# wenhao728/VORTA

Measured on AMD Instinct MI355X. Metric: video_tokens_per_sec (routed-attention denoising step, HunyuanVideo 720p 129f), higher is better.
Workload: dtype fp16

## Files before the change

include/vorta_hip.h:

```cpp
#ifndef VORTA_HIP_H
#define VORTA_HIP_H

#include <stdint.h>

#ifdef __cplusplus
extern "C" {
#endif

#define VORTA_OK 0
#define VORTA_EINVAL (-1)
#define VORTA_EUNSUPPORTED (-2)
#define VORTA_ELAUNCH (-3)

#define VORTA_ABI_VERSION 9

typedef enum vorta_dtype {
  VORTA_BF16 = 0,
  VORTA_FP16 = 1,
  VORTA_FP32 = 2,
  VORTA_FP8E4M3 = 3,
  VORTA_INT8 = 4
} vorta_dtype;

typedef struct vorta_tensor {
// ... 16 lines not shown
  int32_t n_kv, kv_row_offset;
  const int32_t* kv_rows;
  int64_t kv_rows_stride_h, kv_rows_stride_g;
  const int32_t* dup_rows;
  int64_t dup_rows_stride_h;
  int32_t n_dup_pos, n_dup;
  float scale;
  int32_t block_rows;
  int32_t n_splits;
  float* ws_o;
  float* ws_ml;
  const int32_t* n_kv_dev;
  const int32_t* q_valid_dev;
  int32_t variant;
  int32_t reserved;
  const int32_t* q_block_table;
  int32_t n_q_blocks;
  int32_t reserved2;
} vorta_attn_args;

int vorta_attn_fwd(const vorta_attn_args* args, void* hip_stream);
#define VORTA_MAX_FUSED_LAUNCHES 6
int vorta_attn_fwd_batch(const vorta_attn_args* args, int32_t n, void* hip_stream);
int vorta_attn_plan(const vorta_attn_args* args, int32_t* block_rows, int64_t* n_workgroups, int32_t* kernel_id);
int vorta_attn_workspace_bytes(const vorta_attn_args* args, uint64_t* ws_o_bytes, uint64_t* ws_ml_bytes);

typedef struct vorta_attn_bwd_args {
  uint32_t struct_size;
  int32_t reserved;
  vorta_attn_args fwd;
  vorta_tensor d_o;
  const void* do_scale;
  int64_t do_scale_stride_h;
  vorta_tensor dq, dk, dv;
} vorta_attn_bwd_args;

int vorta_attn_bwd(const vorta_attn_bwd_args* args, void* hip_stream);

typedef struct vorta_attn_bwd_kmajor_args {
  uint32_t struct_size;
  int32_t n_key_lists;
  vorta_attn_bwd_args bwd;
  float* stats;
  int64_t stats_stride_h;
} vorta_attn_bwd_kmajor_args;

// ... 317 lines not shown
```

vorta_amd/_C.py:

```python
import ctypes as C
import os

_HERE = os.path.dirname(os.path.abspath(__file__))
LIB_PATH = os.environ.get("VORTA_HIP_LIB") or os.path.join(_HERE, "csrc", "libvorta_hip.so")

VORTA_OK, VORTA_EINVAL, VORTA_EUNSUPPORTED, VORTA_ELAUNCH = 0, -1, -2, -3
VORTA_BF16, VORTA_FP16, VORTA_FP32, VORTA_FP8E4M3, VORTA_INT8 = 0, 1, 2, 3, 4
ABI_VERSION = 9

_i32, _i64, _u32, _f32, _vp = C.c_int32, C.c_int64, C.c_uint32, C.c_float, C.c_void_p


class Tensor(C.Structure):
    _fields_ = [("ptr", _vp), ("stride_h", _i64), ("stride_s", _i64)]


class AttnArgs(C.Structure):
    _fields_ = [
        ("struct_size", _u32), ("dtype", _i32), ("head_dim", _i32), ("n_heads", _i32),
        ("q", Tensor), ("k", Tensor), ("v", Tensor), ("o", Tensor),
        ("head_list", _vp), ("n_heads_dev", _vp),
        ("n_q", _i32), ("q_group_len", _i32), ("q_row_offset", _i32), ("q_valid", _i32),
        ("q_rows", _vp), ("q_rows_stride_h", _i64),
        ("n_kv", _i32), ("kv_row_offset", _i32),
# ... 162 lines not shown
        ("rows", _vp), ("win", _vp), ("keep_rows", _vp), ("keep_rows_stride_h", _i64),
        ("drop_rows", _vp), ("drop_rows_stride_h", _i64), ("head_list", _vp), ("n_heads_dev", _vp),
    ]


MIX_BWD_PARTS = 64
NORM_ROPE_BWD_PARTS = 1024
FIDELITY_PARTS, FIDELITY_WS_FLOATS = 64, 12


def fidelity_chain(n_rows: int) -> int:
    return ((n_rows + FIDELITY_PARTS - 1) // FIDELITY_PARTS + 15) // 16 + 21

SAMPLED_FIDELITY_PARTS, SAMPLED_FIDELITY_WS_FLOATS, SAMPLED_FIDELITY_ROW_CHAIN = 16, 8, 11


def sampled_fidelity_chain(n_rows: int) -> int:
    return ((n_rows + SAMPLED_FIDELITY_PARTS - 1) // SAMPLED_FIDELITY_PARTS + 15) // 16 + 19


SYMBOLS = {
    "vorta_attn_fwd": (C.c_int, [C.POINTER(AttnArgs), _vp]),
    "vorta_attn_fwd_batch": (C.c_int, [C.POINTER(AttnArgs), _i32, _vp]),
    "vorta_attn_plan": (C.c_int, [C.POINTER(AttnArgs), C.POINTER(_i32), C.POINTER(_i64), C.POINTER(_i32)]),
    "vorta_attn_workspace_bytes": (C.c_int, [C.POINTER(AttnArgs), C.POINTER(C.c_uint64), C.POINTER(C.c_uint64)]),
    "vorta_fp8_quant_ws_floats": (C.c_int, [_i32, _i32]),
    "vorta_fp8_quant_ws_partials": (C.c_int, [_i32, _i32, C.POINTER(_i64), C.POINTER(_i64)]),
    "vorta_fp8_quantize_qkv": (C.c_int, [C.POINTER(Fp8QuantArgs), _vp]),
    "vorta_fp8_v_absmax": (C.c_int, [C.POINTER(Fp8VArgs), _vp]),
    "vorta_fp8_v_convert": (C.c_int, [C.POINTER(Fp8VArgs), _vp]),
    "vorta_attn_fwd_fp8": (C.c_int, [C.POINTER(AttnArgs), C.POINTER(AttnFp8Ext), _vp]),
    "vorta_attn_fwd_batch_fp8": (C.c_int, [C.POINTER(AttnArgs), C.POINTER(AttnFp8Ext), _i32, _vp]),
    "vorta_i8_quantize_k": (C.c_int, [C.POINTER(I8QuantArgs), _vp]),
    "vorta_i8_tail_flags": (C.c_int, [C.POINTER(Tensor), _i32, _i32, _vp, C.c_float, _vp, _vp]),
    "vorta_split_heads": (C.c_int, [_vp, _vp, _i32, _vp, _vp, _vp, _vp, _vp]),
    "vorta_attn_fwd_i8": (C.c_int, [C.POINTER(AttnArgs), C.POINTER(AttnI8Ext), _vp]),
    "vorta_attn_fwd_batch_i8": (C.c_int, [C.POINTER(AttnArgs), C.POINTER(AttnI8Ext), _i32, _vp]),
    "vorta_coreset_select": (C.c_int, [C.POINTER(CoresetArgs), _vp]),
    "vorta_sta_table_sizes": (C.c_int, [C.POINTER(StaArgs), C.POINTER(_i32), C.POINTER(_i32), C.POINTER(_i32)]),
    "vorta_sta_build_tables": (C.c_int, [C.POINTER(StaArgs), _vp]),
    "vorta_coreset_select_partial": (C.c_int, [C.POINTER(CoresetArgs), _vp]),
    "vorta_sta_partial_sizes": (C.c_int, [C.POINTER(StaArgs), C.POINTER(_i32), C.POINTER(_i32), C.POINTER(_i32),
                                          C.POINTER(_i32), _i32]),
    "vorta_sta_build_tables_partial": (C.c_int, [C.POINTER(StaArgs), _vp]),
    "vorta_router_route": (C.c_int, [C.POINTER(RouterArgs), _vp]),
    "vorta_route_scores": (C.c_int, [C.POINTER(RouterArgs), _vp]),
# ... 88 lines not shown
```

vorta_amd/_debug.py:

```python
import os

KEYS = ("coreset_kv_order", "fused_text_splits", "sta_merge", "fp8_center_k", "joint_projection", "attn_variant", "no_xcd_remap",
        "sp_staging", "sp_group_streams", "sp_v_wire", "sp_emulate_link_gbps")


def _parse(text: str) -> dict:
    out = {}
    for item in filter(None, (x.strip() for x in text.split(","))):
        key, _, value = item.partition("=")
        if key not in KEYS:
            raise ValueError(f"VORTA_DEBUG: unknown key {key!r} (one of {KEYS})")
        out[key] = value if value else "1"
    return out


FLAGS = _parse(os.environ.get("VORTA_DEBUG", ""))


def flag(key: str, default: str) -> str:
    if key not in KEYS:
        raise KeyError(key)
    return FLAGS.get(key, default)
```

vorta_amd/csrc/attn_common.h:

```cpp
#pragma once
#include <hip/hip_runtime.h>
#include <stdint.h>

#include "vorta_hip.h"
#include "common.h"

namespace vorta_attn {


constexpr int KVB = 64;
constexpr int D = 128;
constexpr int ROWB = D * 2;
constexpr int TILE_BYTES = KVB * ROWB;
constexpr int BUF_BYTES = 2 * TILE_BYTES;

struct Params {
  const char* q; const char* k; const char* v; char* o;
  int64_t q_sh, k_sh, v_sh, o_sh;
  int64_t q_ss, k_ss, v_ss, o_ss;
  const int32_t* head_list; const int32_t* n_heads_dev;
  int n_heads;
  int n_q, q_group_len, q_row_offset, q_valid;
  int n_groups, blocks_per_group;
  const int32_t* q_rows; int64_t q_rows_sh;
// ... 24 lines not shown
__device__ __forceinline__ int live_order(const Params& p, int b, int n, bool remap) {
  if (p.n_heads_dev) n = min(n, max(*p.n_heads_dev, 0) * p.wg_per_slot);
  if (!remap || b >= n) return b;
  const int xcd = b & 7, qd = n >> 3, r = n & 7;
  return (xcd < r ? xcd * (qd + 1) : r * (qd + 1) + (xcd - r) * qd) + (b >> 3);
}

#ifndef VORTA_MAX_SEGMENTS
#define VORTA_MAX_SEGMENTS VORTA_MAX_FUSED_LAUNCHES
#endif
constexpr int MAX_SEGMENTS = VORTA_MAX_SEGMENTS;
template <class PP> __host__ __device__ __forceinline__ Params& base_of(PP& pp) { return pp.p; }
template <class PP> __host__ __device__ __forceinline__ const Params& base_of(const PP& pp) { return pp.p; }
__host__ __device__ __forceinline__ Params& base_of(Params& p) { return p; }
__host__ __device__ __forceinline__ const Params& base_of(const Params& p) { return p; }

template <class PP> struct MultiOf {
  PP seg[MAX_SEGMENTS];
  int start[MAX_SEGMENTS + 1];
  int n;
};

template <class PP>
__device__ __forceinline__ const PP& segment_of(const MultiOf<PP>& mp, int b, int& wg) {
  int s = 0;
#pragma unroll
  for (int i = 1; i < MAX_SEGMENTS; ++i) s += (i < mp.n && b >= mp.start[i]) ? 1 : 0;
  wg = live_order(base_of(mp.seg[s]), b - mp.start[s], mp.start[s + 1] - mp.start[s], true);
  return mp.seg[s];
}

__device__ __forceinline__ float2 out_descale(const Params&, int, int) { return make_float2(1.f, 1.f); }
template <class PP> __device__ __forceinline__ float2 out_descale(const PP& pp, int head, int lane) {
  return *(const float2*)(pp.v_descale + (int64_t)head * pp.v_descale_sh + lane * 2);
}

template <typename T, class PP>
__global__ __launch_bounds__(256) void attn_combine_kernel(const PP pp) {
  const Params& p = base_of(pp);
  const int lane = threadIdx.x & 63;
  const int64_t item = (int64_t)blockIdx.x * 4 + (threadIdx.x >> 6);
  if (item >= (int64_t)p.n_heads * p.n_q) return;
  const int y = (int)(item / p.n_q);
  const int pos = (int)(item - (int64_t)y * p.n_q);
  if (p.n_heads_dev && y >= *p.n_heads_dev) return;
  const int head = p.head_list ? p.head_list[y] : y;
  float m = -1e30f;
  for (int s = 0; s < p.n_splits; ++s) m = fmaxf(m, p.ws_ml[(((int64_t)y * p.n_splits + s) * p.n_q + pos) * 2]);
  float acc0 = 0.f, acc1 = 0.f, l = 0.f;
  for (int s = 0; s < p.n_splits; ++s) {
    const int64_t slot = ((int64_t)y * p.n_splits + s) * p.n_q + pos;
    const float w = __builtin_amdgcn_exp2f(p.ws_ml[slot * 2] - m);
// ... 36 lines not shown
int launch_single(void (*kernel)(PP), int block_rows, const PP& pp, hipStream_t st) {
  const Params& p = base_of(pp);
  const int64_t total = (int64_t)p.n_groups * p.blocks_per_group * p.n_heads * p.n_splits;
  if (total <= 0) return VORTA_OK;
  if (total > 0x7fffffff) return VORTA_EINVAL;
  hipLaunchKernelGGL(kernel, dim3((unsigned)total), dim3(block_rows * 2), 0, st, pp);
  const hipError_t e = hipGetLastError();
  if (e != hipSuccess) return vorta_set_hip_error(e);
  return launch_combine<T>(pp, st);
}

template <class F>
int fwd_single(const F& f, const vorta_attn_args* a, void* hip_stream) {
  typename F::PP pp{};
  int block_rows = 0;
  const int rc = f.fill(a, pp, block_rows);
  if (rc != VORTA_OK) return rc;
  if (base_of(pp).n_heads == 0 || base_of(pp).n_groups == 0) return VORTA_OK;
  hipStream_t st = (hipStream_t)hip_stream;
  if (f.out_dtype(*a) == VORTA_BF16) return launch_single<__bf16>(F::template kernel<__bf16>(*a, pp, block_rows), block_rows, pp, st);
  return launch_single<_Float16>(F::template kernel<_Float16>(*a, pp, block_rows), block_rows, pp, st);
}

template <typename T, class PP>
int launch_fused(void (*kernel)(MultiOf<PP>), const MultiOf<PP>& mp, int total, hipStream_t st) {
  hipLaunchKernelGGL(kernel, dim3((unsigned)total), dim3(512), 0, st, mp);
  const hipError_t e = hipGetLastError();
  if (e != hipSuccess) return vorta_set_hip_error(e);
  for (int i = 0; i < mp.n; ++i) {
    const int rc = launch_combine<T>(mp.seg[i], st);
    if (rc != VORTA_OK) return rc;
  }
  return VORTA_OK;
}

template <class F>
int fwd_batch(const F& f, const vorta_attn_args* args, int32_t n, void* hip_stream) {
  if (!args || n < 0 || n > MAX_SEGMENTS) return VORTA_EINVAL;
  MultiOf<typename F::PP> mp{};
  int64_t total = 0;
  int dtype = -1, m = 0;
  for (int i = 0; i < n; ++i) {
    typename F::PP pp{};
    int block_rows = 0;
    const int rc = f.fill(&args[i], pp, block_rows);
    if (rc != VORTA_OK) return rc;
    Params& p = base_of(pp);
    if (p.n_heads == 0 || p.n_groups == 0) continue;
    if (block_rows != 256 || !f.fusable(args[i], pp)) return VORTA_EUNSUPPORTED;
    if (dtype >= 0 && dtype != f.out_dtype(args[i])) return VORTA_EINVAL;
    dtype = f.out_dtype(args[i]);
    p.xcd_remap = 0;
    mp.seg[m] = pp;
    mp.start[m] = (int)total;
    total += (int64_t)p.n_groups * p.blocks_per_group * p.n_heads * p.n_splits;
    if (total > 0x7fffffff) return VORTA_EINVAL;
    ++m;
  }
  if (m == 0) return VORTA_OK;
  for (int i = m; i <= MAX_SEGMENTS; ++i) mp.start[i] = (int)total;
  mp.n = m;
  hipStream_t st = (hipStream_t)hip_stream;
  if (dtype == VORTA_BF16) return launch_fused<__bf16>(F::template multi<__bf16>, mp, (int)total, st);
  return launch_fused<_Float16>(F::template multi<_Float16>, mp, (int)total, st);
}

int fill_params(const vorta_attn_args* a, Params& p, int& block_rows, int in_esize, int v_esize = 0, int k_esize = 0);
int mx_fwd(const vorta_attn_args* a, const vorta_attn_fp8_ext* ext, void* hip_stream);
int mx_fwd_batch(const vorta_attn_args* args, const vorta_attn_fp8_ext* ext, int32_t n, void* hip_stream);

template <typename T> struct MF;
template <> struct MF<__bf16> {
  using v8 = bf16x8; using v4 = bf16x4;
  static __device__ __forceinline__ f32x16 mfma(v8 a, v8 b, f32x16 c) {
    return __builtin_amdgcn_mfma_f32_32x32x16_bf16(a, b, c, 0, 0, 0);
  }
  static __device__ __forceinline__ v4 tr(const char* p) {
    return __builtin_amdgcn_ds_read_tr16_b64_v4bf16((LDS_AS v4*)p);
  }
};
template <> struct MF<_Float16> {
  using v8 = f16x8; using v4 = f16x4;
  static __device__ __forceinline__ f32x16 mfma(v8 a, v8 b, f32x16 c) {
    return __builtin_amdgcn_mfma_f32_32x32x16_f16(a, b, c, 0, 0, 0);
  }
  static __device__ __forceinline__ v4 tr(const char* p) {
    typedef __attribute__((ext_vector_type(4))) __fp16 h4;
// ... 17 lines not shown
```

vorta_amd/csrc/attn_fwd.hip:

```cpp
#include <hip/hip_runtime.h>
#include <stdint.h>

#include "vorta_hip.h"
#include "common.h"

#include "attn_common.h"
#include "attn_fwd_diag.inc"

namespace {
using namespace vorta_attn;

template <typename T, int NW>
__global__ __launch_bounds__(NW * 64, 2) void attn_fwd_kernel(const Params p) {
  using V8 = typename MF<T>::v8;
  using V4 = typename MF<T>::v4;
  constexpr int NT = NW * 64;
  constexpr int QB = NW * 32;
  constexpr int CH = (KVB * 16) / NT;
  constexpr int ROWSTEP = NT / 16;

  __shared__ __attribute__((aligned(16))) char smem[2 * BUF_BYTES];

  const int wg = live_order(p, blockIdx.x, gridDim.x, p.xcd_remap);
  const int sp = wg % p.n_splits;
  const int rest = wg / p.n_splits;
  const int n_qb = p.n_groups * p.blocks_per_group;
  const int qb = rest % n_qb;
  const int y = rest / n_qb;
  if (p.n_heads_dev && y >= *p.n_heads_dev) return;
  const int head = p.head_list ? p.head_list[y] : y;
  int grp, p0, pend;
  q_block_of(p, qb, QB, grp, p0, pend);

  const int tid = threadIdx.x;
  const int lane = tid & 63;
  const int wave = __builtin_amdgcn_readfirstlane(tid >> 6);
  const int r32 = lane & 31;
  const int hh = lane >> 5;

  const int n_kv = p.n_kv_dev ? max(1, min(*p.n_kv_dev, p.n_kv)) : p.n_kv;
  const int q_valid = p.q_valid_dev ? min(*p.q_valid_dev, p.q_valid) : p.q_valid;
  const int nblk_total = (n_kv + KVB - 1) / KVB;
  const int blk0 = sp * p.blocks_per_split;
  const int blk1 = min(blk0 + p.blocks_per_split, nblk_total);

  const int wrow0 = p0 + wave * 32;
  const bool wave_active = wrow0 < pend;
  const int my_p = wrow0 + r32;
  const bool row_ok = my_p < pend;
  const int ld_p = min(my_p, pend - 1);
  const int32_t* q_rows = p.q_rows ? p.q_rows + (int64_t)y * p.q_rows_sh : nullptr;
  const int64_t my_row = q_rows ? (int64_t)q_rows[ld_p] : (int64_t)(p.q_row_offset + ld_p);

  V8 qf[8];
  {
    const char* qp = p.q + (int64_t)head * p.q_sh + my_row * p.q_ss + hh * 16;
#pragma unroll
    for (int ks = 0; ks < 8; ++ks) qf[ks] = *(const V8*)(qp + ks * 32);
  }

  const int32_t* kv_rows =
      p.kv_rows ? p.kv_rows + (int64_t)y * p.kv_rows_sh + (int64_t)grp * p.kv_rows_sg : nullptr;
  const char* kbase = p.k + (int64_t)head * p.k_sh + (tid & 15) * 16;
  const char* vbase = p.v + (int64_t)head * p.v_sh + (tid & 15) * 16;
  const int lrow0 = tid >> 4;
  const int lcc = tid & 15;
  int k_wr[CH], v_wr[CH];
#pragma unroll
  for (int i = 0; i < CH; ++i) {
    const int row = lrow0 + i * ROWSTEP;
// ... 31 lines not shown

  f32x16 o[4];
#pragma unroll
  for (int dt = 0; dt < 4; ++dt)
#pragma unroll
    for (int i = 0; i < 16; ++i) o[dt][i] = 0.f;
  float m_run = -1e30f, l_run = 0.f;
  const float c = p.scale_log2;

  if (blk0 < blk1) {
    FETCH_ROWS(blk0);
    ISSUE_LOADS();
    if (blk0 + 1 < blk1) { FETCH_ROWS(blk0 + 1); }
    WRITE_LDS(0);
    if (blk0 + 1 < blk1) { ISSUE_LOADS(); }
    if (blk0 + 2 < blk1) { FETCH_ROWS(blk0 + 2); }
    __syncthreads();
  }

  for (int blk = blk0; blk < blk1; ++blk) {
    const int buf = (blk - blk0) & 1;
    const char* sb = smem + buf * BUF_BYTES;
    V8 pb[4];
    if (wave_active) {
      f32x16 s0, s1;
#pragma unroll
      for (int i = 0; i < 16; ++i) { s0[i] = 0.f; s1[i] = 0.f; }
#pragma unroll
      for (int ks = 0; ks < 8; ++ks) {
        const V8 k0 = *(const V8*)(sb + k_rd[ks]);
        const V8 k1 = *(const V8*)(sb + k_rd[ks] + 32 * ROWB);
        s0 = MF<T>::mfma(k0, qf[ks], s0);
        s1 = MF<T>::mfma(k1, qf[ks], s1);
      }
      const int kv0 = blk * KVB;
      if (kv0 + KVB > n_kv) {
#pragma unroll
        for (int i = 0; i < 16; ++i) {
          const int row = (i & 3) + 8 * (i >> 2) + 4 * hh;
          if (kv0 + row >= n_kv) s0[i] = -INFINITY;
          if (kv0 + 32 + row >= n_kv) s1[i] = -INFINITY;
        }
      }
      float mx = s0[0];
#pragma unroll
      for (int i = 1; i < 16; ++i) mx = fmaxf(mx, s0[i]);
#pragma unroll
// ... 11 lines not shown
      }
      const float mc = m_run * c;
      float lsum = 0.f;
#pragma unroll
      for (int i = 0; i < 16; ++i) {
        s0[i] = __builtin_amdgcn_exp2f(fmaf(s0[i], c, -mc));
        s1[i] = __builtin_amdgcn_exp2f(fmaf(s1[i], c, -mc));
        lsum += s0[i] + s1[i];
      }
      l_run += lsum;
#pragma unroll
      for (int j = 0; j < 8; ++j) {
        pb[0][j] = (T)s0[j];
        pb[1][j] = (T)s0[8 + j];
        pb[2][j] = (T)s1[j];
        pb[3][j] = (T)s1[8 + j];
      }
    }
    if (blk + 1 < blk1) {
      WRITE_LDS(buf ^ 1);
      if (blk + 2 < blk1) { ISSUE_LOADS(); }
      if (blk + 3 < blk1) { FETCH_ROWS(blk + 3); }
    }
    if (wave_active) {
#pragma unroll
      for (int dt = 0; dt < 4; ++dt) {
#pragma unroll
        for (int kg = 0; kg < 4; ++kg) {
          const V4 lo = MF<T>::tr(sb + v_rd[dt] + (16 * kg) * ROWB);
          const V4 hi = MF<T>::tr(sb + v_rd[dt] + (16 * kg + 8) * ROWB);
          V8 vf;
#pragma unroll
          for (int j = 0; j < 4; ++j) { vf[j] = lo[j]; vf[4 + j] = hi[j]; }
          o[dt] = MF<T>::mfma(vf, pb[kg], o[dt]);
        }
      }
    }
    __syncthreads();
  }

  if (!wave_active) return;
  const float l_tot = half_sum(l_run);
  if (p.n_splits > 1) {
    if (row_ok) {
      const int64_t slot = ((int64_t)y * p.n_splits + sp) * p.n_q + my_p;
      float* wo = p.ws_o + slot * D;
#pragma unroll
// ... 40 lines not shown

constexpr int RING = 2;

template <typename T, int NW, bool KVTAB, int NS>
__device__ __forceinline__ void attn_pipe_dma_body(const Params& p, char* __restrict__ smem, const int wg) {
  static_assert(NS == 2, "ring depth");
  TRACE_ENTRY_()
  using V8 = typename MF<T>::v8;
  using V4 = typename MF<T>::v4;
  constexpr int NT = NW * 64;
  constexpr int QB = NW * 32;
  constexpr int CH = (KVB * 16) / NT;
  constexpr int ROWSTEP = NT / 16;
#ifndef VORTA_KPRE
#define VORTA_KPRE 2
#endif
  constexpr int KPRE = (NW == 4 && KVTAB && VORTA_KPRE > 1) ? 1 : VORTA_KPRE;
  const int sp = wg % p.n_splits;
  const int rest = wg / p.n_splits;
  const int n_qb = p.n_groups * p.blocks_per_group;
  const int qb = rest % n_qb;
  const int y = rest / n_qb;
  if (p.n_heads_dev && y >= *p.n_heads_dev) return;
  const int head = p.head_list ? p.head_list[y] : y;
  int grp, p0, pend;
  q_block_of(p, qb, QB, grp, p0, pend);

  const int tid = threadIdx.x;
  const int lane = tid & 63;
  const int wave = __builtin_amdgcn_readfirstlane(tid >> 6);
  const int r32 = lane & 31;
  const int hh = lane >> 5;

  const int n_kv = p.n_kv_dev ? max(1, min(*p.n_kv_dev, p.n_kv)) : p.n_kv;
  const int q_valid = p.q_valid_dev ? min(*p.q_valid_dev, p.q_valid) : p.q_valid;
  const int nblk_total = (n_kv + KVB - 1) / KVB;
  const int blk0 = sp * p.blocks_per_split;
  const int blk1 = min(blk0 + p.blocks_per_split, nblk_total);

  const int wrow0 = p0 + wave * 32;
  const bool wave_active = wrow0 < pend;
  const int my_p = wrow0 + r32;
  const int ld_p = min(my_p, pend - 1);
  const int32_t* q_rows = p.q_rows ? p.q_rows + (int64_t)y * p.q_rows_sh : nullptr;
  const int64_t my_row = q_rows ? (int64_t)q_rows[ld_p] : (int64_t)(p.q_row_offset + ld_p);

  V8 qf[8];
  {
    const char* qp = p.q + (int64_t)head * p.q_sh + my_row * p.q_ss + hh * 16;
#pragma unroll
    for (int ks = 0; ks < 8; ++ks) {
      const V8 raw = *(const V8*)(qp + ks * 32);
#pragma unroll
      for (int i = 0; i < 8; ++i) qf[ks][i] = (T)((float)raw[i] * p.scale_log2);
    }
  }

  const int32_t* kv_rows =
      p.kv_rows ? p.kv_rows + (int64_t)y * p.kv_rows_sh + (int64_t)grp * p.kv_rows_sg : nullptr;
  const char* kbase = p.k + (int64_t)head * p.k_sh + (tid & 15) * 16;
  const char* vbase = p.v + (int64_t)head * p.v_sh + (tid & 15) * 16;
  const int lrow0 = tid >> 4;
  const int lcc = tid & 15;
  const __amdgpu_buffer_rsrc_t k_rsrc = __builtin_amdgcn_make_buffer_rsrc(
// ... 137 lines not shown
#define SCHED_RECIPE()                                                            \
  _Pragma("unroll") for (int g_ = 0; g_ < 16; ++g_) {                             \
    __builtin_amdgcn_sched_group_barrier(0x008, 1, 0);                            \
    __builtin_amdgcn_sched_group_barrier(0x100, 1, 0);                            \
    __builtin_amdgcn_sched_group_barrier(0x400, 2, 0);                            \
    __builtin_amdgcn_sched_group_barrier(0x002, 2, 0);                            \
  }                                                                               \
  _Pragma("unroll") for (int g_ = 0; g_ < 16; ++g_) {                             \
    __builtin_amdgcn_sched_group_barrier(0x008, 1, 0);                            \
    __builtin_amdgcn_sched_group_barrier(0x100, 2, 0);                            \
    __builtin_amdgcn_sched_group_barrier(0x002, 4, 0);                            \
  }
#else
#define SCHED_RECIPE()
#endif
#define STEP(c0_, c1_, n0_, n1_, kcur_, knext_, vfree_, j_, tail_)                \
  {  \
    STAGE_DMA(kcur_, vfree_, j_, tail_)                                           \
    STEP_BODY(c0_, c1_, n0_, n1_, kcur_, knext_, j_, tail_)                       \
    STEP_SYNC()                                                                   \
  }
#define STEP_BODY(c0_, c1_, n0_, n1_, kcur_, knext_, j_, tail_)                   \
  {                                                                               \
    if (wave_active) {                                                            \
      V8 kpre_[KPRE > 0 ? KPRE : 1][2];                                                          \
      _Pragma("unroll") for (int ks_ = 0; ks_ < KPRE; ++ks_) {                    \
        kpre_[ks_][0] = *(const V8*)(smem + (knext_) * TILE_BYTES + k_rd[ks_]);   \
        kpre_[ks_][1] = *(const V8*)(smem + (knext_) * TILE_BYTES + k_rd[ks_] + 32 * ROWB); \
      }                                                                           \
       \
       \
      if ((tail_) && (j_) * KVB + KVB > n_kv) {                                   \
        int h4_ = 4 * hh;  \
        asm volatile("" : "+v"(h4_));                                             \
        _Pragma("unroll") for (int i_ = 0; i_ < 16; ++i_) {                       \
          const int row_ = (i_ & 3) + 8 * (i_ >> 2) + h4_;                        \
          if ((j_) * KVB + row_ >= n_kv) c0_[i_] = -INFINITY;                     \
          if ((j_) * KVB + 32 + row_ >= n_kv) c1_[i_] = -INFINITY;                \
        }                                                                         \
        ROW_MAX(mx_cur, c0_, c1_)                                                 \
      }                                                                           \
       \
       \
       \
      if (!__all(mx_cur <= defer)) {                                              \
        const float g_ = fmaxf(mx_cur, 0.f);                                      \
        RAISE_REF(g_, c0_, c1_)                                                   \
// ... 21 lines not shown
          _Pragma("unroll") for (int e_ = 0; e_ < 4; ++e_) { vf_[e_] = lo_[e_]; vf_[4 + e_] = hi_[e_]; } \
          o[dt_] = MF<T>::mfma(vf_, pb_[kg_], o[dt_]);                            \
        }                                                                         \
      }                                                                           \
      ROW_MAX_POS(mx_cur, n0_, n1_)  \
      SCHED_RECIPE()                                                              \
    }                                                                             \
  }

  if (blk0 < blk1) {
    ROWS_OF(rowK, blk0, true)
    _Pragma("unroll") for (int i_ = 0; i_ < CH; ++i_) rowV[i_] = rowK[i_];
    DMA_K(0)
    DMA_V(0)
    ROWS_OF(rowK, blk0 + 1, true)
    DMA_K(1)
    _Pragma("unroll") for (int i_ = 0; i_ < CH; ++i_) rowV[i_] = rowK[i_];
    ROWS_OF(rowK, blk0 + NS, true)
    _Pragma("unroll") for (int i_ = 0; i_ < CH; ++i_) posK[i_] = (blk0 + NS) * KVB + 4 * (CH * wave + i_) + (lane >> 4);
    if constexpr (!KVTAB) {
      _Pragma("unroll") for (int i_ = 0; i_ < CH; ++i_) { offK[i_] = (unsigned)K_OFF(i_); offV[i_] = (unsigned)V_OFF(i_); }
    }
    __syncthreads();
    if (wave_active) {
      QK(sA0, sA1, 0)
      if (blk0 * KVB + KVB > n_kv) {
#pragma unroll
        for (int i = 0; i < 16; ++i) {
          const int row = (i & 3) + 8 * (i >> 2) + 4 * hh;
          if (blk0 * KVB + row >= n_kv) sA0[i] = -INFINITY;
          if (blk0 * KVB + 32 + row >= n_kv) sA1[i] = -INFINITY;
        }
      }
      ROW_MAX(mx_cur, sA0, sA1)
      m_run = mx_cur;
#pragma unroll
      for (int i = 0; i < 16; ++i) { sA0[i] -= m_run; sA1[i] -= m_run; minit[i] = -m_run; }
      asm volatile("" : "+v"(minit));
      mx_cur = 0.f;
    }
    __syncthreads();
  }
  const int blk_whole = min(blk1, n_kv / KVB - (KVTAB ? NS + 1 : NS));
  int blk = blk0;
  for (; blk + 1 < blk_whole; blk += 2) {
    STEP(sA0, sA1, sB0, sB1, 0, 1, 1, blk, false)
    STEP(sB0, sB1, sA0, sA1, 1, 0, 0, blk + 1, false)
// ... 8 lines not shown
  for (; blk < blk1; blk += 2) {
    STEP(sA0, sA1, sB0, sB1, 0, 1, 1, blk, true)
    if (blk + 1 >= blk1) break;
    STEP(sB0, sB1, sA0, sA1, 1, 0, 0, blk + 1, true)
  }
#undef QK
#undef QK_PRE
#undef ROW_MAX
#undef ROW_MAX_POS
#undef RAISE_REF
#undef STEP
#undef STEP_BODY
#undef STAGE_DMA
#undef STEP_SYNC
#undef ROWS_OF
#undef DMA_K
#undef DMA_V
#undef DMA_K_AT
#undef DMA_V_AT
#undef K_OFF
#undef V_OFF

  TRACE_FLUSH_()
  if (!wave_active) return;
  int tid_e = threadIdx.x;
  asm volatile("" : "+v"(tid_e));
  const int hh_e = (tid_e >> 5) & 1;
  const int e_p = wrow0 + (tid_e & 31);
  const bool e_ok = e_p < pend;
  const int64_t e_row = q_rows ? (int64_t)q_rows[min(e_p, pend - 1)] : (int64_t)(p.q_row_offset + min(e_p, pend - 1));
  const float l_tot = half_sum(l_run);
  if (p.n_splits > 1) {
    if (e_ok) {
      const int64_t slot = ((int64_t)y * p.n_splits + sp) * p.n_q + e_p;
      float* wo = p.ws_o + slot * D;
#pragma unroll
      for (int dt = 0; dt < 4; ++dt)
#pragma unroll
        for (int rg = 0; rg < 4; ++rg) {
          f32x4 v = {o[dt][4 * rg], o[dt][4 * rg + 1], o[dt][4 * rg + 2], o[dt][4 * rg + 3]};
          *(f32x4*)(wo + 32 * dt + 8 * rg + 4 * hh_e) = v;
        }
      if (hh_e == 0) {
        p.ws_ml[slot * 2] = m_run;
        p.ws_ml[slot * 2 + 1] = l_tot;
      }
    }
// ... 20 lines not shown
#pragma unroll
      for (int rg = 0; rg < 4; ++rg) *(uint2*)(op + (32 * dt + 8 * rg) * 2) = packed[dt * 4 + rg];
  };
  store_row(e_row);
  if (p.dup_rows && e_p < p.n_dup_pos) {
    const int32_t* dr = p.dup_rows + (int64_t)y * p.dup_rows_sh + (int64_t)e_p * p.n_dup;
    for (int i = 0; i < p.n_dup; ++i) store_row((int64_t)dr[i]);
  }
}


template <typename T, int NW, bool KVTAB>
__global__ __launch_bounds__(NW * 64, 2) void attn_fwd_pipe_kernel(const Params p) {
#if defined(__HIP_DEVICE_COMPILE__)
  constexpr int NS = RING;
  __shared__ __attribute__((aligned(16))) char smem[2 * NS * TILE_BYTES];
  const int wg = live_order(p, blockIdx.x, gridDim.x, p.xcd_remap);
  attn_pipe_dma_body<T, NW, KVTAB, NS>(p, smem, wg);
#endif
}


template <typename T>
__global__ __launch_bounds__(512, 2) void attn_fwd_multi_kernel(const MultiOf<Params> mp) {
#if defined(__HIP_DEVICE_COMPILE__)
  __shared__ __attribute__((aligned(16))) char smem[2 * RING * TILE_BYTES];
  int wg;
  const Params& p = segment_of(mp, blockIdx.x, wg);
  if (p.kv_rows) attn_pipe_dma_body<T, 8, true, RING>(p, smem, wg);
  else attn_pipe_dma_body<T, 8, false, RING>(p, smem, wg);
#endif
}

}

int vorta_attn::fill_params(const vorta_attn_args* a, Params& p, int& block_rows, int in_esize, int v_esize, int k_esize) {
  if (v_esize == 0) v_esize = in_esize;
  if (k_esize == 0) k_esize = in_esize;
  if (!a || a->struct_size != sizeof(vorta_attn_args)) return VORTA_EINVAL;
  if (in_esize == 2 ? (a->dtype != VORTA_BF16 && a->dtype != VORTA_FP16) : a->dtype != VORTA_FP8E4M3) return VORTA_EUNSUPPORTED;
  if (a->head_dim != D) return VORTA_EUNSUPPORTED;
  if (a->n_heads < 0 || a->n_q < 0 || a->n_kv < 0) return VORTA_EINVAL;
  if (a->n_heads == 0 || a->n_q == 0) { block_rows = 0; p.n_groups = 0; p.blocks_per_group = 0; p.n_heads = 0; return VORTA_OK; }
  if (a->n_kv == 0) return VORTA_EINVAL;
  if (!a->q.ptr || !a->k.ptr || !a->v.ptr || !a->o.ptr) return VORTA_EINVAL;
  const vorta_tensor* ts[4] = {&a->q, &a->k, &a->v, &a->o};
  for (int i = 0; i < 4; ++i) {
    const vorta_tensor* t = ts[i];
    const int al = 16 / (i == 0 ? in_esize : i == 1 ? k_esize : i == 2 ? v_esize : 2);
    if (((uintptr_t)t->ptr & 15) || (t->stride_s % al) || (t->stride_h % al) || t->stride_s < D) return VORTA_EINVAL;
  }
  if (a->n_splits < 1 || a->n_splits > 1024) return VORTA_EINVAL;
  if (!(a->scale > 0.f)) return VORTA_EINVAL;
// ... 66 lines not shown
  if (a->n_splits <= 1) { *ws_o_bytes = 0; *ws_ml_bytes = 0; return VORTA_OK; }
  const uint64_t slots = (uint64_t)a->n_heads * (uint64_t)a->n_splits * (uint64_t)a->n_q;
  *ws_o_bytes = slots * D * sizeof(float);
  *ws_ml_bytes = slots * 2 * sizeof(float);
  return VORTA_OK;
}

extern "C" int vorta_attn_plan(const vorta_attn_args* a, int32_t* block_rows_out, int64_t* n_workgroups_out,
                               int32_t* kernel_id_out) {
  Params p{};
  int block_rows = 0;
  int rc = vorta_attn::fill_params(a, p, block_rows, (a && a->dtype == VORTA_FP8E4M3) ? 1 : 2);
  if (rc != VORTA_OK) return rc;
  if (block_rows_out) *block_rows_out = block_rows;
  if (kernel_id_out) {
    const bool pipe = a->variant != 1;
    *kernel_id_out = (block_rows == 256 ? 8 : 4) * 16 + (pipe ? 1 : 0) + ((pipe && a->kv_rows) ? 2 : 0);
  }
  if (n_workgroups_out) *n_workgroups_out = (int64_t)p.n_groups * p.blocks_per_group * p.n_heads * (p.n_heads ? p.n_splits : 0);
  return VORTA_OK;
}

extern "C" int vorta_attn_fwd_batch(const vorta_attn_args* args, int32_t n, void* hip_stream) {
  return fwd_batch(Family16{}, args, n, hip_stream);
}

extern "C" int vorta_attn_fwd(const vorta_attn_args* a, void* hip_stream) { return fwd_single(Family16{}, a, hip_stream); }
```

vorta_amd/csrc/attn_fwd_diag.inc:

```
#ifdef VORTA_TRACE
#define TRACE_ENTRY_() const long long tr_e0_ = wall_clock64();
#define TRACE_VARS_()                                                             \
  long long tr_wait_ = 0, tr_bar_ = 0;                                            \
  const long long tr_t0_ = clock64();                                             \
  const long long tr_w0_ = wall_clock64();
#define STEP_SYNC()                                                               \
  {                                                                               \
    const long long a_ = clock64();                                               \
    asm volatile("s_waitcnt vmcnt(0) lgkmcnt(0)" ::: "memory");                   \
    const long long b_ = clock64();                                               \
    asm volatile("s_barrier" ::: "memory");                                       \
    const long long c_ = clock64();                                               \
    tr_wait_ += b_ - a_;                                                          \
    tr_bar_ += c_ - b_;                                                           \
  }
#define TRACE_FLUSH_()                                                            \
  if (p.n_splits == 1 && p.ws_ml && lane == 0) {                                  \
    long long* tr = (long long*)p.ws_ml + ((int64_t)wg * NW + wave) * 8;          \
    tr[0] = clock64() - tr_t0_; tr[1] = tr_wait_; tr[2] = tr_bar_; tr[3] = blk1 - blk0; \
    tr[4] = wall_clock64() - tr_w0_;                                              \
    tr[5] = tr_e0_; tr[6] = wall_clock64();   \
    tr[7] = (long long)__builtin_amdgcn_s_getreg((4 << 0) | (0 << 6) | (31 << 11)) |    \
            ((long long)__builtin_amdgcn_s_getreg((20 << 0) | (0 << 6) | (31 << 11)) << 32);   \
  }
#else
#define TRACE_ENTRY_()
#define TRACE_VARS_()
#define TRACE_FLUSH_()
#endif
```

vorta_amd/ops.py:

```python
from __future__ import annotations

import ctypes as C
import math
from typing import NamedTuple, Optional, Sequence, Tuple

import torch

from . import _C

_DT = {torch.bfloat16: _C.VORTA_BF16, torch.float16: _C.VORTA_FP16}
FP8_STORAGE = torch.uint8


class Timeline:

    def __init__(self):
        self.records = []

    def summary(self):
        torch.cuda.synchronize()
        out = {}
        for tag, br, nwg, flops, e0, e1 in self.records:
            d = out.setdefault((tag, br), dict(launches=0, ms=0.0, flops=0.0, workgroups=0))
            d["launches"] += 1
            d["ms"] += e0.elapsed_time(e1)
            d["flops"] += flops
            d["workgroups"] += nwg
        return out


_timeline: Optional[Timeline] = None
from ._debug import flag as _debug_flag
DEFAULT_VARIANT = int(_debug_flag("attn_variant", "0"))
NO_XCD_REMAP = int(_debug_flag("no_xcd_remap", "0"))


def set_timeline(t: Optional[Timeline]):
    global _timeline
    _timeline = t


def _stream() -> int:
    return torch.cuda.current_stream().cuda_stream


def _require_gpu(*ts: torch.Tensor):
    for t in ts:
        if t is not None and not t.is_cuda:
            raise _C.VortaHipError("vorta_amd ops need tensors on an MI355X (cuda) device; there is no CPU path")


def _tensor(t: torch.Tensor) -> _C.Tensor:
    if t.dim() != 3 or t.stride(2) != 1:
        raise ValueError(f"expected a (H,S,D) view with contiguous D, got shape {tuple(t.shape)} strides {t.stride()}")
    return _C.Tensor(t.data_ptr(), t.stride(0), t.stride(1))


# ... 45 lines not shown
        if qp is None or qp.dtype != torch.float32 or qp.dim() != 3 or tuple(qp.shape[1:]) != (2, q.shape[-1]) \
                or not qp.is_contiguous() or hs is None or hs.dtype != torch.float32 or not hs.is_contiguous():
            raise ValueError("int8-score attention needs i8.q_prep (heads, 2, D) and i8.k_head_scale (heads,) float32 from i8_quantize_k")
    if fp8:
        if not (k.dtype == v.dtype == FP8_STORAGE) or out.dtype not in _DT:
            raise ValueError("fp8 attention takes e4m3 (uint8) q,k,v and a bf16 / fp16 output")
    elif mixed:
        if q.dtype not in _DT or not (q.dtype == k.dtype == out.dtype):
            raise ValueError("mixed-precision attention takes 16-bit q, k, out of one dtype and an e4m3 (uint8) v")
    elif i8:
        pass
    elif q.dtype not in _DT or not (q.dtype == k.dtype == v.dtype == out.dtype):
        raise ValueError("q,k,v,out must share dtype bf16 or fp16")
    if fp8 or mixed or i8:
        if v_descale is None or v_descale.dtype != torch.float32 or v_descale.dim() != 2 or v_descale.shape[1] != q.shape[-1] \
                or not v_descale.is_contiguous():
            raise ValueError("fp8 attention needs v_descale: contiguous float32 (heads, D) from fp8_quantize_qkv / fp8_quantize_v")
    a = _C.AttnArgs()
    a.struct_size = C.sizeof(_C.AttnArgs)
    a.dtype = _C.VORTA_FP8E4M3 if fp8 else _DT[q.dtype]
    a._ext = None
    a._family = _FAMILIES["i8" if i8 else "fp8" if fp8 else "mx" if mixed else "16"]
    a._out_type = "_Float16" if out.dtype == torch.float16 else "__bf16"
    if i8:
        ext = _C.AttnI8Ext()
        ext.struct_size = C.sizeof(_C.AttnI8Ext)
        ext.k_bias, ext.k_bias_stride_h = i8ops.k_bias.data_ptr(), i8ops.k_bias.stride(0)
        ext.q_prep, ext.q_prep_stride_h = i8ops.q_prep.data_ptr(), i8ops.q_prep.stride(0)
        ext.k_head_scale = i8ops.k_head_scale.data_ptr()
        a._i8ops = i8ops
        ext.v_descale, ext.v_descale_stride_h = v_descale.data_ptr(), v_descale.stride(0)
        o = fp8_opts or FP8_OPTS
        ext.p_bias, ext.defer = float(o.get("p_bias", 0.0)), float(o.get("defer", 0.0))
        a._ext = ext
    elif fp8 or mixed:
        ext = _C.AttnFp8Ext()
        ext.struct_size = C.sizeof(_C.AttnFp8Ext)
        ext.out_dtype = _DT[out.dtype]
        ext.v_descale, ext.v_descale_stride_h = v_descale.data_ptr(), v_descale.stride(0)
        o = fp8_opts or FP8_OPTS
        ext.p_bias, ext.defer, ext.flags = float(o.get("p_bias", 0.0)), float(o.get("defer", 0.0)), int(o.get("flags", 0))
        if mixed:
            ext.flags |= 2
        a._ext = ext
    a.head_dim = q.shape[-1]
    a.q, a.k, a.v, a.o = _tensor(q), _tensor(k), _tensor(v), _tensor(out)
# ... 156 lines not shown
        fused = sorted((i for i in range(len(built)) if in_grid[i]), key=lambda i: (not hints[i][1], i))
        attn_fwd_batch_built([built[i] for i in fused])
        attn_fwd_batch_built([b for b, g in zip(built, in_grid) if not g], fuse=False)
        return
    attn_fwd_batch_built(built, fuse=False)


def attn_fwd_batch_built(built, fuse: bool = True) -> None:
    if not (fuse and len(built) > 1):
        for a, ws, tag, flops in built:
            _timed(lambda: _launch_one(a), tag, flops, [a])
        return
    args = [a for a, _, _, _ in built]
    fam = args[0]._family
    if any(a._family is not fam for a in args):
        raise ValueError("a fused grid is all 16-bit, all e4m3, all mixed-precision or all int8-score")
    if args[0]._ext is not None:
        for i, a in enumerate(args[1:], 1):
            diff = [f for f, _ in a._ext._fields_ if getattr(a._ext, f) != getattr(args[0]._ext, f)]
            if diff:
                raise ValueError(f"fused launch {i} carries other 8-bit operands or options than launch 0 ({', '.join(diff)}): "
                                 "one grid takes one operand set; launch it separately")
    arr = (_C.AttnArgs * len(args))(*args)
    go = lambda: _C.check(getattr(_C.lib(), fam.batch)(arr, *_ext(args[0]), len(args), _stream()), fam.batch)
    _timed(go, "+".join(t for _, _, t, _ in built), sum(f for _, _, _, f in built), args, fam.multi.format(t=args[0]._out_type))


FP8_OPTS: dict = {}


class Fp8Operands:
    __slots__ = ("q", "k", "v", "v_descale", "ws")

    def __init__(self, q, k, v, v_descale, ws):
        self.q, self.k, self.v, self.v_descale, self.ws = q, k, v, v_descale, ws

    def multipliers(self):
        H, D = self.v_descale.shape
        base = 2 * H + H * D
        return self.ws[base:base + H], self.ws[base + H:base + 2 * H], self.ws[base + 2 * H:base + 2 * H + H * D].view(H, D)

    def k_center(self):
        H, D = self.v_descale.shape
        base = 2 * (2 * H + H * D)
        return self.ws[base:base + H * D].view(H, D)


# ... 826 lines not shown
```

Measured before the change: 28910.

## Add atomic ticket scheduling to fused attention grid and skip invalid query rows

New measurement: 30260, median of 6. +4.7%, better.

```diff
diff --git a/include/vorta_hip.h b/include/vorta_hip.h
--- a/include/vorta_hip.h
+++ b/include/vorta_hip.h
@@ -62,6 +62,8 @@
 int vorta_attn_fwd(const vorta_attn_args* args, void* hip_stream);
 #define VORTA_MAX_FUSED_LAUNCHES 6
 int vorta_attn_fwd_batch(const vorta_attn_args* args, int32_t n, void* hip_stream);
+int vorta_attn_fwd_batch_tickets(const vorta_attn_args* args, int32_t n, int32_t* tickets, void* hip_stream);
+int vorta_attn_ticket_workspace_ints(void);
 int vorta_attn_plan(const vorta_attn_args* args, int32_t* block_rows, int64_t* n_workgroups, int32_t* kernel_id);
 int vorta_attn_workspace_bytes(const vorta_attn_args* args, uint64_t* ws_o_bytes, uint64_t* ws_ml_bytes);
 
diff --git a/vorta_amd/_C.py b/vorta_amd/_C.py
--- a/vorta_amd/_C.py
+++ b/vorta_amd/_C.py
@@ -208,6 +208,8 @@
 SYMBOLS = {
     "vorta_attn_fwd": (C.c_int, [C.POINTER(AttnArgs), _vp]),
     "vorta_attn_fwd_batch": (C.c_int, [C.POINTER(AttnArgs), _i32, _vp]),
+    "vorta_attn_fwd_batch_tickets": (C.c_int, [C.POINTER(AttnArgs), _i32, _vp, _vp]),
+    "vorta_attn_ticket_workspace_ints": (C.c_int, []),
     "vorta_attn_plan": (C.c_int, [C.POINTER(AttnArgs), C.POINTER(_i32), C.POINTER(_i64), C.POINTER(_i32)]),
     "vorta_attn_workspace_bytes": (C.c_int, [C.POINTER(AttnArgs), C.POINTER(C.c_uint64), C.POINTER(C.c_uint64)]),
     "vorta_fp8_quant_ws_floats": (C.c_int, [_i32, _i32]),
diff --git a/vorta_amd/_debug.py b/vorta_amd/_debug.py
--- a/vorta_amd/_debug.py
+++ b/vorta_amd/_debug.py
@@ -1,6 +1,6 @@
 import os
 
-KEYS = ("coreset_kv_order", "fused_text_splits", "sta_merge", "fp8_center_k", "joint_projection", "attn_variant", "no_xcd_remap",
+KEYS = ("coreset_kv_order", "fused_text_splits", "sta_merge", "fp8_center_k", "joint_projection", "attn_variant", "no_xcd_remap", "fused_tickets",
         "sp_staging", "sp_group_streams", "sp_v_wire", "sp_emulate_link_gbps")
 
 
diff --git a/vorta_amd/csrc/attn_common.h b/vorta_amd/csrc/attn_common.h
--- a/vorta_amd/csrc/attn_common.h
+++ b/vorta_amd/csrc/attn_common.h
@@ -70,12 +70,60 @@
 };
 
 template <class PP>
-__device__ __forceinline__ const PP& segment_of(const MultiOf<PP>& mp, int b, int& wg) {
+__device__ __forceinline__ int segment_index(const MultiOf<PP>& mp, int b, int& wg) {
   int s = 0;
 #pragma unroll
   for (int i = 1; i < MAX_SEGMENTS; ++i) s += (i < mp.n && b >= mp.start[i]) ? 1 : 0;
   wg = live_order(base_of(mp.seg[s]), b - mp.start[s], mp.start[s + 1] - mp.start[s], true);
-  return mp.seg[s];
+  return s;
+}
+template <class PP>
+__device__ __forceinline__ const PP& segment_of(const MultiOf<PP>& mp, int b, int& wg) {
+  return mp.seg[segment_index(mp, b, wg)];
+}
+
+constexpr int TICKET_INTS = 8 * MAX_SEGMENTS + 8;
+static_assert(MAX_SEGMENTS <= 8, "draw_ticket keeps one (segment, class) pair per lane");
+template <class PP>
+__device__ __forceinline__ int draw_ticket(const MultiOf<PP>& mp, int32_t* cnt, int b, int& wg) {
+  const int lane = threadIdx.x & 63;
+  const int x_l = lane & 7;
+  int len_l = 0, base_l = 0;
+#pragma unroll
+  for (int i = 0; i < MAX_SEGMENTS; ++i) {
+    if (i < mp.n) {
+      const Params& p = base_of(mp.seg[i]);
+      int n = mp.start[i + 1] - mp.start[i];
+      if (p.n_heads_dev) n = min(n, max(*p.n_heads_dev, 0) * p.wg_per_slot);
+      const int qd = n >> 3, r = n & 7;
+      if ((lane >> 3) == i) {
+        len_l = qd + (x_l < r ? 1 : 0);
+        base_l = x_l < r ? x_l * (qd + 1) : r * (qd + 1) + (x_l - r) * qd;
+      }
+    }
+  }
+  for (;;) {
+    int left = 0;
+    if (len_l > 0) left = max(len_l - __hip_atomic_load(cnt + lane, __ATOMIC_RELAXED, __HIP_MEMORY_SCOPE_AGENT), 0);
+    int pick;
+    const unsigned long long own = __ballot(left > 0 && x_l == (b & 7));
+    if (own) {
+      pick = __ffsll(own) - 1;
+    } else {
+      int most = left;
+#pragma unroll
+      for (int off = 32; off > 0; off >>= 1) most = max(most, __shfl_xor(most, off));
+      if (most == 0) return -1;
+      pick = __ffsll(__ballot(left == most)) - 1;
+    }
+    int t = 0;
+    if (lane == pick) t = __hip_atomic_fetch_add(cnt + lane, 1, __ATOMIC_RELAXED, __HIP_MEMORY_SCOPE_AGENT);
+    t = __shfl(t, pick);
+    if (t < __shfl(len_l, pick)) {
+      wg = __shfl(base_l, pick) + t;
+      return pick >> 3;
+    }
+  }
 }
 
 __device__ __forceinline__ float2 out_descale(const Params&, int, int) { return make_float2(1.f, 1.f); }
@@ -158,9 +206,29 @@
   return launch_single<_Float16>(F::template kernel<_Float16>(*a, pp, block_rows), block_rows, pp, st);
 }
 
-template <typename T, class PP>
-int launch_fused(void (*kernel)(MultiOf<PP>), const MultiOf<PP>& mp, int total, hipStream_t st) {
-  hipLaunchKernelGGL(kernel, dim3((unsigned)total), dim3(512), 0, st, mp);
+template <int N>
+__global__ void ticket_reset_kernel(int32_t* cnt) {
+  if (threadIdx.x < N) cnt[threadIdx.x] = 0;
+}
+inline int before_grid(hipStream_t) { return VORTA_OK; }
+template <class I>
+int before_grid(hipStream_t st, I* tickets) {
+  if (!tickets) return VORTA_OK;
+  hipLaunchKernelGGL(ticket_reset_kernel<TICKET_INTS>, dim3(1), dim3(64), 0, st, tickets);
+  const hipError_t e = hipGetLastError();
+  return e == hipSuccess ? VORTA_OK : vorta_set_hip_error(e);
+}
+
+inline int grid_blocks(int64_t total) { return (int)total; }
+template <class I>
+int grid_blocks(int64_t total, I* tickets) {
+  if (!tickets) return (int)total;
+  return (int)min((int64_t)0x7fffffff, total + ((total / 8 + 7) & ~(int64_t)7));
+}
+
+template <typename T, class PP, class... X>
+int launch_fused(void (*kernel)(MultiOf<PP>, X...), const MultiOf<PP>& mp, int total, hipStream_t st, X... extra) {
+  hipLaunchKernelGGL(kernel, dim3((unsigned)total), dim3(512), 0, st, mp, extra...);
   const hipError_t e = hipGetLastError();
   if (e != hipSuccess) return vorta_set_hip_error(e);
   for (int i = 0; i < mp.n; ++i) {
@@ -170,8 +238,8 @@
   return VORTA_OK;
 }
 
-template <class F>
-int fwd_batch(const F& f, const vorta_attn_args* args, int32_t n, void* hip_stream) {
+template <class F, class... X>
+int fwd_batch(const F& f, const vorta_attn_args* args, int32_t n, void* hip_stream, X... extra) {
   if (!args || n < 0 || n > MAX_SEGMENTS) return VORTA_EINVAL;
   MultiOf<typename F::PP> mp{};
   int64_t total = 0;
@@ -197,8 +265,11 @@
   for (int i = m; i <= MAX_SEGMENTS; ++i) mp.start[i] = (int)total;
   mp.n = m;
   hipStream_t st = (hipStream_t)hip_stream;
-  if (dtype == VORTA_BF16) return launch_fused<__bf16>(F::template multi<__bf16>, mp, (int)total, st);
-  return launch_fused<_Float16>(F::template multi<_Float16>, mp, (int)total, st);
+  const int rc = before_grid(st, extra...);
+  if (rc != VORTA_OK) return rc;
+  const int blocks = grid_blocks(total, extra...);
+  if (dtype == VORTA_BF16) return launch_fused<__bf16>(F::template multi<__bf16>, mp, blocks, st, extra...);
+  return launch_fused<_Float16>(F::template multi<_Float16>, mp, blocks, st, extra...);
 }
 
 int fill_params(const vorta_attn_args* a, Params& p, int& block_rows, int in_esize, int v_esize = 0, int k_esize = 0);
diff --git a/vorta_amd/csrc/attn_fwd.hip b/vorta_amd/csrc/attn_fwd.hip
--- a/vorta_amd/csrc/attn_fwd.hip
+++ b/vorta_amd/csrc/attn_fwd.hip
@@ -42,10 +42,11 @@
   const int q_valid = p.q_valid_dev ? min(*p.q_valid_dev, p.q_valid) : p.q_valid;
   const int nblk_total = (n_kv + KVB - 1) / KVB;
   const int blk0 = sp * p.blocks_per_split;
-  const int blk1 = min(blk0 + p.blocks_per_split, nblk_total);
+  const int blk1 = p0 >= q_valid ? blk0 : min(blk0 + p.blocks_per_split, nblk_total);
 
   const int wrow0 = p0 + wave * 32;
   const bool wave_active = wrow0 < pend;
+  const bool wave_compute = wave_active && wrow0 < q_valid;
   const int my_p = wrow0 + r32;
   const bool row_ok = my_p < pend;
   const int ld_p = min(my_p, pend - 1);
@@ -123,7 +124,7 @@
     const int buf = (blk - blk0) & 1;
     const char* sb = smem + buf * BUF_BYTES;
     V8 pb[4];
-    if (wave_active) {
+    if (wave_compute) {
       f32x16 s0, s1;
 #pragma unroll
       for (int i = 0; i < 16; ++i) { s0[i] = 0.f; s1[i] = 0.f; }
@@ -181,7 +182,7 @@
       if (blk + 2 < blk1) { ISSUE_LOADS(); }
       if (blk + 3 < blk1) { FETCH_ROWS(blk + 3); }
     }
-    if (wave_active) {
+    if (wave_compute) {
 #pragma unroll
       for (int dt = 0; dt < 4; ++dt) {
 #pragma unroll
@@ -268,9 +269,11 @@
   const int qb = rest % n_qb;
   const int y = rest / n_qb;
   if (p.n_heads_dev && y >= *p.n_heads_dev) return;
-  const int head = p.head_list ? p.head_list[y] : y;
+#define UNI(x_) __builtin_amdgcn_readfirstlane(x_)
+  const int head = p.head_list ? UNI(p.head_list[y]) : y;
   int grp, p0, pend;
   q_block_of(p, qb, QB, grp, p0, pend);
+  grp = UNI(grp); p0 = UNI(p0); pend = UNI(pend);
 
   const int tid = threadIdx.x;
   const int lane = tid & 63;
@@ -278,14 +281,16 @@
   const int r32 = lane & 31;
   const int hh = lane >> 5;
 
-  const int n_kv = p.n_kv_dev ? max(1, min(*p.n_kv_dev, p.n_kv)) : p.n_kv;
-  const int q_valid = p.q_valid_dev ? min(*p.q_valid_dev, p.q_valid) : p.q_valid;
+  const int n_kv = p.n_kv_dev ? max(1, min(UNI(*p.n_kv_dev), p.n_kv)) : p.n_kv;
+  const int q_valid = p.q_valid_dev ? min(UNI(*p.q_valid_dev), p.q_valid) : p.q_valid;
+#undef UNI
   const int nblk_total = (n_kv + KVB - 1) / KVB;
   const int blk0 = sp * p.blocks_per_split;
-  const int blk1 = min(blk0 + p.blocks_per_split, nblk_total);
+  const int blk1 = p0 >= q_valid ? blk0 : min(blk0 + p.blocks_per_split, nblk_total);
 
   const int wrow0 = p0 + wave * 32;
   const bool wave_active = wrow0 < pend;
+  const bool wave_compute = wave_active && wrow0 < q_valid;
   const int my_p = wrow0 + r32;
   const int ld_p = min(my_p, pend - 1);
   const int32_t* q_rows = p.q_rows ? p.q_rows + (int64_t)y * p.q_rows_sh : nullptr;
@@ -469,7 +474,7 @@
   }
 #define STEP_BODY(c0_, c1_, n0_, n1_, kcur_, knext_, j_, tail_)                   \
   {                                                                               \
-    if (wave_active) {                                                            \
+    if (wave_compute) {                                                           \
       V8 kpre_[KPRE > 0 ? KPRE : 1][2];                                                          \
       _Pragma("unroll") for (int ks_ = 0; ks_ < KPRE; ++ks_) {                    \
         kpre_[ks_][0] = *(const V8*)(smem + (knext_) * TILE_BYTES + k_rd[ks_]);   \
@@ -537,7 +542,7 @@
       _Pragma("unroll") for (int i_ = 0; i_ < CH; ++i_) { offK[i_] = (unsigned)K_OFF(i_); offV[i_] = (unsigned)V_OFF(i_); }
     }
     __syncthreads();
-    if (wave_active) {
+    if (wave_compute) {
       QK(sA0, sA1, 0)
       if (blk0 * KVB + KVB > n_kv) {
 #pragma unroll
@@ -592,7 +597,9 @@
 #undef V_OFF
 
   TRACE_FLUSH_()
-  if (!wave_active) return;
+  int wrow0_e = wrow0;
+  asm volatile("" : "+v"(wrow0_e));
+  if (__builtin_amdgcn_readfirstlane(wrow0_e) >= pend) return;
   int tid_e = threadIdx.x;
   asm volatile("" : "+v"(tid_e));
   const int hh_e = (tid_e >> 5) & 1;
@@ -659,13 +666,29 @@
 
 
 template <typename T>
-__global__ __launch_bounds__(512, 2) void attn_fwd_multi_kernel(const MultiOf<Params> mp) {
+__global__ __launch_bounds__(512, 2) void attn_fwd_multi_kernel(const MultiOf<Params> mp, int32_t* tickets) {
 #if defined(__HIP_DEVICE_COMPILE__)
   __shared__ __attribute__((aligned(16))) char smem[2 * RING * TILE_BYTES];
-  int wg;
-  const Params& p = segment_of(mp, blockIdx.x, wg);
+  int wg, s;
+  if (tickets) {
+    int* drawn = (int*)smem;
+    if (threadIdx.x < 64) {
+      int w;
+      const int sg = draw_ticket(mp, tickets, blockIdx.x, w);
+      if (threadIdx.x == 0) { drawn[0] = sg; drawn[1] = w; }
+    }
+    __syncthreads();
+    s = __builtin_amdgcn_readfirstlane(drawn[0]);
+    wg = __builtin_amdgcn_readfirstlane(drawn[1]);
+    __syncthreads();
+    if (s < 0) return;
+  } else {
+    s = segment_index(mp, blockIdx.x, wg);
+  }
+  const Params& p = mp.seg[s];
   if (p.kv_rows) attn_pipe_dma_body<T, 8, true, RING>(p, smem, wg);
   else attn_pipe_dma_body<T, 8, false, RING>(p, smem, wg);
+  TRACE_WG_END_(p, wg)
 #endif
 }
 
@@ -778,7 +801,14 @@
 }
 
 extern "C" int vorta_attn_fwd_batch(const vorta_attn_args* args, int32_t n, void* hip_stream) {
-  return fwd_batch(Family16{}, args, n, hip_stream);
+  return fwd_batch(Family16{}, args, n, hip_stream, (int32_t*)nullptr);
+}
+
+extern "C" int vorta_attn_ticket_workspace_ints(void) { return TICKET_INTS; }
+
+extern "C" int vorta_attn_fwd_batch_tickets(const vorta_attn_args* args, int32_t n, int32_t* tickets, void* hip_stream) {
+  if ((uintptr_t)tickets & 3) return VORTA_EINVAL;
+  return fwd_batch(Family16{}, args, n, hip_stream, tickets);
 }
 
 extern "C" int vorta_attn_fwd(const vorta_attn_args* a, void* hip_stream) { return fwd_single(Family16{}, a, hip_stream); }
diff --git a/vorta_amd/csrc/attn_fwd_diag.inc b/vorta_amd/csrc/attn_fwd_diag.inc
--- a/vorta_amd/csrc/attn_fwd_diag.inc
+++ b/vorta_amd/csrc/attn_fwd_diag.inc
@@ -23,8 +23,18 @@
     tr[7] = (long long)__builtin_amdgcn_s_getreg((4 << 0) | (0 << 6) | (31 << 11)) |    \
             ((long long)__builtin_amdgcn_s_getreg((20 << 0) | (0 << 6) | (31 << 11)) << 32);   \
   }
+#define TRACE_WG_END_(p_, wg_)                                                    \
+  if ((p_).n_splits == 1 && (p_).ws_ml && (threadIdx.x & 63) == 0) {              \
+    asm volatile("s_waitcnt vmcnt(0)" ::: "memory");                              \
+    long long* te_ = (long long*)(p_).ws_ml + (int64_t)(p_).n_heads * (p_).wg_per_slot * 64 + \
+                     ((int64_t)(wg_) * 8 + (threadIdx.x >> 6)) * 2;               \
+    te_[0] = wall_clock64();                                                      \
+    te_[1] = (long long)__builtin_amdgcn_s_getreg((4 << 0) | (0 << 6) | (31 << 11)) |    \
+             ((long long)__builtin_amdgcn_s_getreg((20 << 0) | (0 << 6) | (31 << 11)) << 32);   \
+  }
 #else
 #define TRACE_ENTRY_()
 #define TRACE_VARS_()
 #define TRACE_FLUSH_()
+#define TRACE_WG_END_(p_, wg_)
 #endif
diff --git a/vorta_amd/ops.py b/vorta_amd/ops.py
--- a/vorta_amd/ops.py
+++ b/vorta_amd/ops.py
@@ -33,6 +33,16 @@
 from ._debug import flag as _debug_flag
 DEFAULT_VARIANT = int(_debug_flag("attn_variant", "0"))
 NO_XCD_REMAP = int(_debug_flag("no_xcd_remap", "0"))
+FUSED_TICKETS = int(_debug_flag("fused_tickets", "1"))
+_ticket_ws: dict = {}
+
+
+def _tickets(device: torch.device) -> int:
+    key = (device.index, _stream())
+    ws = _ticket_ws.get(key)
+    if ws is None:
+        ws = _ticket_ws[key] = torch.zeros(_C.lib().vorta_attn_ticket_workspace_ints(), dtype=torch.int32, device=device)
+    return ws.data_ptr()
 
 
 def set_timeline(t: Optional[Timeline]):
@@ -124,6 +134,7 @@
     a._ext = None
     a._family = _FAMILIES["i8" if i8 else "fp8" if fp8 else "mx" if mixed else "16"]
     a._out_type = "_Float16" if out.dtype == torch.float16 else "__bf16"
+    a._device = out.device
     if i8:
         ext = _C.AttnI8Ext()
         ext.struct_size = C.sizeof(_C.AttnI8Ext)
@@ -326,7 +337,12 @@
                 raise ValueError(f"fused launch {i} carries other 8-bit operands or options than launch 0 ({', '.join(diff)}): "
                                  "one grid takes one operand set; launch it separately")
     arr = (_C.AttnArgs * len(args))(*args)
-    go = lambda: _C.check(getattr(_C.lib(), fam.batch)(arr, *_ext(args[0]), len(args), _stream()), fam.batch)
+    if fam is _FAMILIES["16"] and FUSED_TICKETS:
+        tickets = _tickets(built[0][0]._device)
+        go = lambda: _C.check(_C.lib().vorta_attn_fwd_batch_tickets(arr, len(args), tickets, _stream()),
+                              "vorta_attn_fwd_batch_tickets")
+    else:
+        go = lambda: _C.check(getattr(_C.lib(), fam.batch)(arr, *_ext(args[0]), len(args), _stream()), fam.batch)
     _timed(go, "+".join(t for _, _, t, _ in built), sum(f for _, _, _, f in built), args, fam.multi.format(t=args[0]._out_type))
 
 
```
